# jedisct1/zig-lz4

Measured on AMD Instinct MI355X. Metric: GiB/s uncompressed, block compress+decompress, higher is better.
Workload: dtype u8

## Files before the change

### zig-lz4_amd/csrc/zlz4_compress_dict.hip

```cpp
#include "zlz4_device.hpp"
#include "zlz4_launch.hpp"

namespace zlz4 {

namespace {

__device__ __forceinline__ uint32_t dc_hash4(uint32_t seq) { return (seq * kHashMul) >> 20; }

__device__ __forceinline__ uint32_t dc_skip_sum(uint32_t x) {
    const uint32_t q = x >> 6, r = x & 63u;
    return 32u * q * (q - 1u) + q * r;
}

__device__ __forceinline__ int64_t dc_last_literals(uint8_t *dst, uint32_t dst_len, uint32_t op, const uint8_t *lit_src,
                                                    uint32_t lit, uint32_t lane) {
    if (lit == 0) return (int64_t)op;
    const uint32_t nle = ext_len_bytes(lit);
    if ((uint64_t)op + 1u + nle + lit > dst_len) return kErrOutputTooSmall;
    if (lane == 0) dst[op] = (uint8_t)((lit >= 15u ? 15u : lit) << 4);
    if (lit >= 15u) write_ext_len(dst + op + 1u, lit, lane);
    copy_bytes(dst + op + 1u + nle, lit_src, lit, lane);
    return (int64_t)(op + 1u + nle + lit);
}

// ... 16 lines not shown
    __device__ __forceinline__ uint32_t rd32(uint32_t p) const {
        if (whole(p, 4u)) return ld32(at(p));
        return (uint32_t)byte(p) | (uint32_t)byte(p + 1u) << 8 | (uint32_t)byte(p + 2u) << 16 | (uint32_t)byte(p + 3u) << 24;
    }
};

__device__ __forceinline__ uint32_t dc_extend_match(const VBuf &V, uint32_t m_pos, uint32_t m_cand, uint32_t mlen,
                                                    uint32_t match_limit, uint32_t lane) {
    const uint32_t ip0 = m_pos + kMinMatch, mt0 = m_cand + kMinMatch;
    for (;;) {
        const uint32_t p = ip0 + mlen + lane * 16u;
        uint32_t n = 0;
        if (p < match_limit) n = (match_limit - p) < 16u ? (match_limit - p) : 16u;
        uint32_t d = 0;
        if (n > 0) {
            const uint32_t q = mt0 + mlen + lane * 16u;
            if (p + 16u <= V.end && V.whole(q, 16u)) {
                d = first_diff16(ld128(V.srcv + p), ld128(V.at(q)));
                if (d > n) d = n;
            } else {
                while (d < n && V.srcv[p + d] == V.byte(q + d)) d++;
            }
        }
        const uint64_t stop = ballot(d < 16u);
        if (stop) {
            const uint32_t sl = first_lane(stop);
            return mlen + sl * 16u + rdlane(d, sl);
        }
        mlen += 1024u;
    }
}

}

template <typename T>
__global__ __launch_bounds__(64) void k_compress_fast_dict(
    const uint8_t *d_in, const uint64_t *__restrict__ d_in_off, const uint32_t *__restrict__ d_in_len,
    uint8_t *__restrict__ d_out, const uint64_t *__restrict__ d_out_off, const uint32_t *__restrict__ d_out_cap,
    const uint8_t *d_dict, const uint64_t *__restrict__ d_dict_off, const uint32_t *__restrict__ d_dict_len,
    const uint32_t *__restrict__ d_table, const uint32_t *__restrict__ d_table_idx, int64_t *__restrict__ d_result,
    uint32_t nblocks, uint32_t max_in_len, uint32_t max_dict_len, uint32_t acceleration) {
    extern __shared__ __attribute__((aligned(16))) uint8_t lds_raw[];
    const uint32_t lane = threadIdx.x & 63u;
    const uint32_t blk = blockIdx.x;
    if (blk >= nblocks) return;
    typedef __attribute__((address_space(3))) volatile T lds_entry;
    lds_entry *table = (lds_entry *)lds_raw;

    const uint8_t *src = d_in + d_in_off[blk];
    uint8_t *dst = d_out + d_out_off[blk];
    const uint32_t src_size = rfl(d_in_len[blk]);
    const uint32_t dst_len = rfl(d_out_cap[blk]);
    const uint32_t dict_len = rfl(d_dict_len[blk]);
    const uint32_t D = dict_len < 65536u ? dict_len : 65536u;

    int64_t res;
    if (src_size > kMaxInput) {
        res = kErrInputTooLarge;
    } else if (src_size > max_in_len || D > max_dict_len) {
        res = kErrInvalidState;
    } else if (src_size == 0) {
        res = 0;
    } else if (src_size < kMfLimit + 1u) {
        res = dc_last_literals(dst, dst_len, 0, src, src_size, lane);
    } else {
        VBuf V;
        V.tail = D ? d_dict + d_dict_off[blk] + (dict_len - D) : src;
        V.srcv = src - D;
        V.D = D;
        V.end = D + src_size;
        const uint32_t L = V.end - kMfLimit;
        const uint32_t match_limit = V.end - kLastLiterals;
        {
            const uint32_t tix = d_table_idx ? rfl(d_table_idx[blk]) : blk;
            const u32x4 *seed4 = reinterpret_cast<const u32x4 *>(d_table + (uint64_t)tix * 4096u);
            for (uint32_t k = lane; k < 1024u; k += 64u) {
                const u32x4 v = seed4[k];
                table[4u * k + 0u] = (T)(v.x < L ? v.x : 0u);
                table[4u * k + 1u] = (T)(v.y < L ? v.y : 0u);
                table[4u * k + 2u] = (T)(v.z < L ? v.z : 0u);
                table[4u * k + 3u] = (T)(v.w < L ? v.w : 0u);
            }
            __builtin_amdgcn_fence(__ATOMIC_RELEASE, "wavefront");
        }
        const uint32_t accel = acceleration < 1u ? 1u : (acceleration > 65537u ? 65537u : acceleration);
        const uint32_t cbase = accel > 64u ? accel : 64u;
        const uint32_t s_cbase = dc_skip_sum(cbase);
        const uint64_t lane_bit = 1ull << lane;
        const uint64_t lanes_below = lane_bit - 1ull;

        uint32_t anchor = D, op = 0;
        uint32_t F0 = D > 1u ? D : 1u;
        bool has_ins = false;
        bool failed = false;
        uint32_t guard = 0;
        u32x4 fwd_pf = {0, 0, 0, 0};
        uint32_t pf_anchor = 0xFFFFFFFFu;
        while (F0 < L) {
            if (++guard > src_size) { failed = true; break; }
            int32_t ub = has_ins ? -1 : 0;

            if (accel == 1u && F0 == anchor + 1u && has_ins && (uint64_t)anchor + 192u < L) {
              bool moved = false;
              bool to_generic = false;
              for (;;) {
                const uint32_t A = anchor;
                const uint32_t pos = A + lane;
                const u32x4 fwd = pf_anchor == A ? fwd_pf : ld128(V.srcv + pos);
                const uint32_t prod = fwd.x * kHashMul;
                const uint32_t h = prod >> 20;
                const uint32_t mine = (uint32_t)(T)pos;
                const uint32_t old = table[h];
                const uint64_t okm = ballot(old > 0) & ballot(old < pos) & ballot(old + kMaxDist >= pos);
                const bool old_ok = in_mask(okm);
                u32x4 cold = {0, 0, 0, 0};
                if (old_ok) cold = V.ld128v(old);
                u32x4 f2 = {0, 0, 0, 0}, c2 = f2, f3 = f2, c3 = f2;
                table[h] = (T)mine;
                __builtin_amdgcn_fence(__ATOMIC_RELEASE, "wavefront");
                const uint32_t rb = table[h];
                uint64_t losers = ballot(rb != mine);
                uint64_t grp = lane_bit;
                while (losers) {
                    const uint32_t l = first_lane(losers);
                    const uint32_t hh = rdlane(h, l);
                    const uint64_t same = ballot(h == hh);
                    if (in_mask(same)) grp = same;
                    losers &= ~same;
                }

                const uint64_t vom = okm & ballot(cold.x == fwd.x);
                const bool vo = in_mask(vom);
                uint32_t mlo;
                {
                    const uint32_t x1 = fwd.y ^ cold.y, x2 = fwd.z ^ cold.z, x3 = fwd.w ^ cold.w;
                    const uint32_t xs = x1 ? x1 : (x2 ? x2 : x3);
                    const uint32_t xbase = x1 ? 0u : (x2 ? 4u : 8u);
                    mlo = xs ? xbase + ((uint32_t)__builtin_ctz(xs) >> 3) : 12u;
                }
                const bool need2 = in_mask(vom & ballot(mlo == 12u));
                if (need2) {
                    f2 = ld128(V.srcv + pos + 16u); f3 = ld128(V.srcv + pos + 32u);
                    c2 = V.ld128v(old + 16u); c3 = V.ld128v(old + 32u);
                }
                if (need2) {
                    const uint32_t d2 = first_diff16_sel(f2, c2);
                    mlo += d2 == 16u ? 16u + first_diff16_sel(f3, c3) : d2;
                }
                const uint64_t singm = ballot(lane_rank(grp) == 0u);
                const uint64_t lt44 = ballot(mlo < 44u);
                const uint64_t cfast = vom & lt44;
                const uint64_t nsing = ~singm;
                const uint64_t slow = (nsing & ~cfast) | (vom & ~lt44);
                uint32_t J, S;
                {
                    const uint64_t mj = cfast >> lane, ms = slow >> lane;
                    J = mj ? lane + (uint32_t)__builtin_ctzll(mj) : 64u;
                    S = ms ? lane + (uint32_t)__builtin_ctzll(ms) : 64u;
                }
                uint32_t v_end = lane + kMinMatch + mlo;
                uint32_t mlo_e = mlo, off_e = pos - old;
                uint32_t XP, Q;
                {
                    const uint32_t xm = J < S ? J : S;
                    XP = xm | ((uint32_t)((nsing >> (xm & 63u)) & 1ull) << 7);
                    Q = (vo ? 1u : 0u) | (mlo << 1);
                }
                uint32_t PK;
                {
                    const uint32_t jc = J & 63u;
                    const uint32_t ve_j = shfl(v_end, jc);
                    const bool fastok = J < 64u && S > J && !((nsing >> jc) & 1ull);
                    PK = fastok ? (J | (ve_j << 6)) : 0xFFFFFFFFu;
                }

                uint32_t f = 1;
                uint32_t a = 0;
                uint32_t nseq = 0;
                uint64_t cov_acc = 0;
                bool continue_generic = false;
                const bool tight = dst_len - op < 512u;
                uint32_t a0 = a, op0 = op;
                uint64_t mm_run = 0;
                auto covered_now = [&]() -> uint64_t {
                    if (mm_run == 0) return cov_acc;
                    const uint64_t mb = mm_run & lanes_below;
                    const uint32_t pj = mb ? 63u - (uint32_t)__builtin_clzll(mb) : 0u;
                    const uint32_t pe = shfl(v_end, pj);
                    return cov_acc | ballot(mb != 0 && lane < pe);
                };
                auto flush_run = [&]() {
                    const uint64_t mb = mm_run & lanes_below;
                    const bool has_prev = mb != 0;
                    const uint32_t pj = has_prev ? 63u - (uint32_t)__builtin_clzll(mb) : 0u;
                    const uint32_t pend_all = shfl(v_end, pj);
                    const uint32_t pend = has_prev ? pend_all : a0;
                    const uint64_t covm = ballot(mb != 0) & ballot(lane < pend_all);
                    const bool is_m = in_mask(mm_run);
                    const uint32_t jlast = 63u - (uint32_t)__builtin_clzll(mm_run);
                    const uint64_t litmask = ballot(lane >= a0) & ~(ballot(lane >= jlast) | covm | mm_run);
                    const bool is_lit = in_mask(litmask);
                    const uint64_t extm = mm_run & ballot(mlo_e >= 15u);
                    const uint64_t at_or_above = mm_run & ~lanes_below;
                    const uint32_t my_m = at_or_above ? (uint32_t)__builtin_ctzll(at_or_above) : lane;
                    const uint64_t ownm = ballot(my_m - pend >= 15u);
                    const uint32_t own_l = in_mask(ownm) ? 1u : 0u;
                    const uint64_t lextm = mm_run & ownm;
                    const uint32_t k = lane_rank(mm_run);
                    const uint32_t lb = lane_rank(litmask);
                    const uint32_t o1 = op0 + 3u * k + lb + 1u + lane_rank(extm) + lane_rank(lextm) + own_l;
                    if (is_lit) dst[o1] = (uint8_t)fwd.x;
                    if (is_m) {
                        const uint32_t lit_k = lane - pend;
                        uint8_t *tk = dst + (o1 - 1u - lit_k - own_l);
                        tk[0] = (uint8_t)(((lit_k < 15u ? lit_k : 15u) << 4) | (mlo_e < 15u ? mlo_e : 15u));
                        if (own_l) tk[1] = (uint8_t)(lit_k - 15u);
                        const uint16_t off16 = (uint16_t)off_e;
                        __builtin_memcpy(dst + o1, &off16, 2);
                        if (mlo_e >= 15u) dst[o1 + 2u] = (uint8_t)(mlo_e - 15u);
                    }
                    const uint32_t nm = (uint32_t)__popcll(mm_run);
                    op = op0 + 3u * nm + (uint32_t)__popcll(litmask) + (uint32_t)__popcll(extm) + (uint32_t)__popcll(lextm);
                    cov_acc |= covm;
                    mm_run = 0;
                };
                for (;;) {
                    if (mm_run == 0) { a0 = a; op0 = op; }
                    if (!tight) {
                        uint32_t t_pk, t_j;
#define ZLZ4_FAST_RUN_TRIP                                   \
                            "s_cmp_gt_u32 %[f], 63\n\t"      \
                            "s_cbranch_scc1 3f\n\t"          \
                            "v_readlane_b32 %[pk], %[PK], %[f]\n\t" \
                            "s_cmp_eq_u32 %[pk], -1\n\t"     \
                            "s_cbranch_scc1 3f\n\t"          \
                            "s_lshr_b32 %[a], %[pk], 6\n\t"  \
                            "s_add_u32 %[f], %[a], 1\n\t"    \
                            "s_and_b32 %[j], %[pk], 63\n\t"  \
                            "s_bitset1_b64 %[mm], %[j]\n\t"  \
                            "s_add_u32 %[nseq], %[nseq], 1\n\t"
                        asm volatile(
                            "s_nop 3\n"
                            "1:\n\t"
                            ZLZ4_FAST_RUN_TRIP
                            ZLZ4_FAST_RUN_TRIP
                            "s_branch 1b\n"
                            "3:\n"
                            : [f] "+s"(f), [a] "+s"(a), [nseq] "+s"(nseq), [mm] "+s"(mm_run), [pk] "=&s"(t_pk), [j] "=&s"(t_j)
                            : [PK] "v"(PK)
                            : "scc");
#undef ZLZ4_FAST_RUN_TRIP
                    }
                    if (f >= 64u) {
                        if (nseq == 0u) continue_generic = true;
                        break;
                    }

                    const uint32_t xp = rdlane(XP, f);
                    const uint32_t x = xp & 127u;
                    if (x >= 64u) {
                        if (nseq == 0u) continue_generic = true;
                        break;
                    }
                    uint64_t pm = 0;
                    if (xp >> 7) {
                        const uint64_t grp_x = (uint64_t)rdlane((uint32_t)grp, x) | ((uint64_t)rdlane((uint32_t)(grp >> 32), x) << 32);
                        pm = grp_x & ~covered_now() & ((1ull << x) - 1ull);
                    }
                    const uint32_t j = x;
                    const uint32_t m_pos = A + j;
                    uint32_t m_cand, mlen;
                    if (pm) {
                        const uint32_t pr = 63u - (uint32_t)__builtin_clzll(pm);
                        if (rdlane(fwd.x, pr) != rdlane(fwd.x, x)) { f = x + 1u; continue; }
                        m_cand = A + pr;
                        const uint64_t xa = ((uint64_t)(rdlane(fwd.z, j) ^ rdlane(fwd.z, pr)) << 32) | (rdlane(fwd.y, j) ^ rdlane(fwd.y, pr));
                        const uint32_t xb = rdlane(fwd.w, j) ^ rdlane(fwd.w, pr);
                        if (xa) mlen = (uint32_t)__builtin_ctzll(xa) >> 3;
                        else if (xb) mlen = 8u + ((uint32_t)__builtin_ctz(xb) >> 3);
                        else mlen = dc_extend_match(V, m_pos, m_cand, 12u, match_limit, lane);
                    } else {
                        const uint32_t q = rdlane(Q, x);
                        if (!(q & 1u)) { f = x + 1u; continue; }
                        mlen = q >> 1;
                        if (mlen < 44u && !tight) {
                            mm_run |= 1ull << j;
                            nseq++;
                            a = j + kMinMatch + mlen;
                            if (a >= 64u) break;
                            f = a + 1u;
                            continue;
                        }
                        m_cand = rdlane(old, x);
                        if (mlen >= 44u) mlen = dc_extend_match(V, m_pos, m_cand, 44u, match_limit, lane);
                    }
                    const uint32_t lit = j - a;
                    const uint32_t offset = m_pos - m_cand;
                    const uint32_t e = j + kMinMatch + mlen;
                    if (!tight && mlen < 270u) {
                        v_end = wrlane(e, j, v_end);
                        mlo_e = wrlane(mlen, j, mlo_e);
                        off_e = wrlane(offset, j, off_e);
                        mm_run |= 1ull << j;
                        nseq++;
                        a = e;
                        if (e >= 64u) break;
                        f = e + 1u;
                        continue;
                    }
                    if (mm_run) flush_run();
                    const uint32_t nle = ext_len_bytes(lit), nme = ext_len_bytes(mlen);
                    const uint64_t seq_end = (uint64_t)op + 1u + nle + lit + 2u + nme;
                    if (seq_end > dst_len) { failed = true; break; }
                    if (lane == 0)
                        dst[op] = (uint8_t)(((lit >= 15u ? 15u : lit) << 4) | (mlen >= 15u ? 15u : mlen));
                    if (lit >= 15u) write_ext_len(dst + op + 1u, lit, lane);
                    uint8_t *o = dst + op + 1u + nle;
                    if (lane >= a && lane < j) o[lane - a] = (uint8_t)fwd.x;
                    o += lit;
                    if (lane < 2u) o[lane] = (uint8_t)(offset >> (8u * lane));
                    if (mlen >= 15u) write_ext_len(o + 2u, mlen, lane);
                    op = (uint32_t)seq_end;
                    {
                        const uint64_t upto_e = e >= 64u ? ~0ull : (1ull << e) - 1ull;
                        cov_acc |= upto_e & ~((2ull << j) - 1ull);
                    }
                    nseq++;
                    a = e;
                    if (e >= 64u) break;
                    f = e + 1u;
                }
                const bool next_win = !continue_generic && !failed && a != 0u && (uint64_t)A + a + 192u < L;
                if (next_win) {
                    pf_anchor = A + a;
                    fwd_pf = ld128(V.srcv + pf_anchor + lane);
                }
                if (mm_run && !failed) flush_run();
                anchor = A + a;
                const uint32_t f_end = continue_generic ? 64u : (a >= 64u ? 64u : a + 1u);
                const uint64_t ins = ~cov_acc & (f_end >= 64u ? ~0ull : (1ull << f_end) - 1ull);
                if (failed) break;
                const uint64_t gi = grp & ins;
                const bool put_mine = in_mask(ins) && (gi & ~lanes_below & ~lane_bit) == 0;
                if (put_mine || gi == 0) table[h] = (T)(put_mine ? mine : old);
                __builtin_amdgcn_fence(__ATOMIC_RELEASE, "wavefront");
                moved = anchor != A;
                to_generic = continue_generic;
                if (next_win) {
                    has_ins = true;
                    F0 = anchor + 1u;
                    continue;
                }
                break;
              }
                if (failed) break;
                if (!to_generic && moved) {
                    if (anchor < L) { has_ins = true; F0 = anchor + 1u; }
                    else { has_ins = false; F0 = L; }
                    continue;
                }
                if (to_generic) ub = 63;
            }

            bool found = false;
            uint32_t m_pos = 0, m_cand = 0, m_local = 0;
            bool m_local_done = false;
            for (;;) {
                const int32_t u = ub + (int32_t)lane;
                uint32_t pos, step_next;
                if (u <= 0) {
                    pos = (u < 0) ? F0 - 1u : F0;
                    step_next = accel;
                } else if (u == 1) {
                    pos = F0 + accel;
                    step_next = accel >> 6;
                } else {
                    const uint32_t x = cbase + (uint32_t)u - 1u;
                    pos = F0 + accel + dc_skip_sum(x) - s_cbase;
                    step_next = x >> 6;
                }
                const bool is_probe = u >= 0;
                const bool bail = is_probe && ((uint64_t)pos + step_next > L);
                const uint64_t bail_mask = ballot(bail);
                const uint32_t nb = bail_mask ? first_lane(bail_mask) : 64u;
                const bool active = lane < nb;

                const bool have16 = active && (pos + 16u <= V.end);
                u32x4 fwd = {0, 0, 0, 0};
                if (have16) fwd = ld128(V.srcv + pos);
                else if (active) fwd.x = ld32(V.srcv + pos);
                const uint32_t h = dc_hash4(fwd.x);
                const uint32_t mine = (uint32_t)(T)pos;

                uint32_t old = 0, rb = 0;
                if (active) {
                    old = table[h];
                    table[h] = (T)mine;
                }
                __builtin_amdgcn_fence(__ATOMIC_RELEASE, "wavefront");
                if (active) rb = table[h];
                uint64_t losers = ballot(active && rb != mine);
                uint64_t grp = lane_bit;
                int32_t pred = -1;
                while (losers) {
                    const uint32_t l = first_lane(losers);
                    const uint32_t hh = rdlane(h, l);
                    const uint64_t same = ballot(active && h == hh);
                    if (active && h == hh) {
                        grp = same;
                        const uint64_t below = same & lanes_below;
                        pred = below ? 63 - (int32_t)__clzll((long long)below) : -1;
                    }
                    losers &= ~same;
                }
                const uint32_t pred_pos = shfl(pos, (uint32_t)(pred < 0 ? 0 : pred));
                const uint32_t cand = pred >= 0 ? pred_pos : old;

                bool valid = is_probe && active && cand > 0 && cand < pos && (cand + kMaxDist >= pos);
                u32x4 cnd = {0, 0, 0, 0};
                bool cnd16 = false;
                if (valid) {
                    cnd16 = have16 && V.whole(cand, 16u);
                    if (cnd16) cnd = ld128(V.at(cand)); else cnd.x = V.rd32(cand);
                    valid = cnd.x == fwd.x;
                }
                const uint64_t valid_mask = ballot(valid);

                if (valid_mask) {
                    const uint32_t wl = first_lane(valid_mask);
                    if (active && lane > wl) table[h] = (T)old;
                    __builtin_amdgcn_fence(__ATOMIC_RELEASE, "wavefront");
                    const uint64_t upto = (2ull << wl) - 1ull;
                    if (active && lane <= wl && ((grp & upto & ~lanes_below & ~lane_bit) == 0)) table[h] = (T)mine;
                    __builtin_amdgcn_fence(__ATOMIC_RELEASE, "wavefront");
                    uint32_t loc = 0;
                    bool loc_done = false;
                    if (lane == wl && cnd16) {
                        const uint32_t lim = match_limit - (pos + kMinMatch);
                        u32x4 a = fwd, b = cnd;
                        a.x = 0; b.x = 0;
                        loc = first_diff16(a, b) - 4u;
                        if (loc >= lim) { loc = lim; loc_done = true; }
                        else if (loc < 12u) loc_done = true;
                    }
                    m_pos = rdlane(pos, wl);
                    m_cand = rdlane(cand, wl);
                    m_local = rdlane(loc, wl);
                    m_local_done = rdlane((uint32_t)loc_done, wl) != 0;
                    found = true;
                    break;
                }
                if (bail_mask) break;
                if (active && ((grp & ~lanes_below & ~lane_bit) == 0) && grp != lane_bit) table[h] = (T)mine;
                __builtin_amdgcn_fence(__ATOMIC_RELEASE, "wavefront");
                ub += 64;
            }
            if (!found) break;

            const uint32_t mlen = m_local_done ? m_local : dc_extend_match(V, m_pos, m_cand, m_local, match_limit, lane);

            const uint32_t lit = m_pos - anchor;
            const uint32_t nle = ext_len_bytes(lit), nme = ext_len_bytes(mlen);
            const uint64_t seq_end = (uint64_t)op + 1u + nle + lit + 2u + nme;
            if (seq_end > dst_len) { failed = true; break; }
            if (lane == 0)
                dst[op] = (uint8_t)(((lit >= 15u ? 15u : lit) << 4) | (mlen >= 15u ? 15u : mlen));
            if (lit >= 15u) write_ext_len(dst + op + 1u, lit, lane);
            uint8_t *o = dst + op + 1u + nle;
            copy_bytes(o, V.srcv + anchor, lit, lane);
            o += lit;
            const uint32_t offset = m_pos - m_cand;
            if (lane < 2u) o[lane] = (uint8_t)(offset >> (8u * lane));
            if (mlen >= 15u) write_ext_len(o + 2u, mlen, lane);
            op = (uint32_t)seq_end;

            const uint32_t end = m_pos + kMinMatch + mlen;
            anchor = end;
            if (end < L) { has_ins = true; F0 = end + 1u; }
            else { has_ins = false; F0 = L; }
        }
// ... 27 lines not shown
```

### zig-lz4_amd/csrc/zlz4_compress_fast.hip

```cpp
#include <cstdlib>

#include "zlz4_device.hpp"
#include "zlz4_launch.hpp"

#ifdef ZLZ4_STAMPS
__device__ unsigned long long g_zlz4_stamps[24];
#define STAMP_DECL unsigned long long st_acc[24] = {0,0,0,0,0,0,0,0,0,0,0,0,0,0,0,0,0,0,0,0,0,0,0,0}; unsigned long long st_last = __builtin_amdgcn_s_memtime();
#define STAMP(i) do { unsigned long long st_now; __builtin_amdgcn_sched_barrier(0); \
                      asm volatile("s_memtime %0\n\ts_waitcnt lgkmcnt(0)" : "=s"(st_now) :: "memory"); \
                      __builtin_amdgcn_sched_barrier(0); st_acc[i] += st_now - st_last; st_last = st_now; } while (0)
#define STAMP_COUNT(i) do { st_acc[i] += 1; } while (0)
#define STAMP_FLUSH do { if (lane == 0) for (int st_k = 0; st_k < 24; st_k++) atomicAdd(&g_zlz4_stamps[st_k], st_acc[st_k]); } while (0)
#else
#define STAMP_DECL
#define STAMP(i)
#define STAMP_COUNT(i)
#define STAMP_FLUSH
#endif

namespace zlz4 {

__device__ __forceinline__ uint32_t hash4(uint32_t seq) { return (seq * kHashMul) >> 20; }

__device__ __forceinline__ uint32_t skip_sum(uint32_t x) {
// ... 98 lines not shown
        const uint32_t cbase = accel > 64u ? accel : 64u;
        const uint32_t s_cbase = skip_sum(cbase);
        const uint32_t L = src_size - kMfLimit;
        const uint32_t match_limit = src_size - kLastLiterals;
        const uint64_t lane_bit = 1ull << lane;
        const uint64_t lanes_below = lane_bit - 1ull;

        uint32_t anchor = 0, op = 0;
        uint32_t F0 = 1;
        bool has_ins = false;
        bool failed = false;
        STAMP_DECL
        STAMP(0);

        uint32_t guard = 0;

        constexpr bool kRing = sizeof(T) == 2;
        uint32_t rpos = 0x80000000u + 4u * lane;
        uint32_t r0 = 0, r1 = 0, r2 = 0;
        uint32_t ring_lim = 0;
        if constexpr (kRing) asm volatile("v_mov_b32 %0, %1" : "=v"(ring_lim) : "s"(src_size - 4u));
        auto ring_q = [&](uint32_t q) -> uint32_t { return q < ring_lim ? q : ring_lim; };
        auto ring_sel = [&](uint32_t A, uint32_t &ja) -> uint32_t {
            uint32_t rel = rfl(A - rpos);
            if (rel >= 256u) {
                const bool reload = rel >= 512u;
                const uint32_t nb = reload ? (A & ~127u) + 4u * lane : rpos + 256u;
                asm volatile("s_waitcnt vmcnt(0)\n\t"
                             "s_cmpk_lt_u32 %[rel], 0x200\n\t"
                             "s_cbranch_scc1 1f\n\t"
                             "global_load_dword %[r0], %[q0], %[src]\n\t"
                             "global_load_dword %[r1], %[q1], %[src]\n\t"
                             "s_waitcnt vmcnt(0)\n\t"
                             "s_branch 2f\n"
                             "1:\n\t"
                             "v_mov_b32 %[r0], %[r1]\n\t"
                             "v_mov_b32 %[r1], %[r2]\n"
                             "2:\n\t"
                             "global_load_dword %[r2], %[q2], %[src]"
                             : [r0] "+v"(r0), [r1] "+v"(r1), [r2] "+v"(r2)
                             : [rel] "s"(rel), [q0] "v"(ring_q(nb)), [q1] "v"(ring_q(nb + 256u)), [q2] "v"(ring_q(nb + 512u)),
                               [src] "s"(src)
                             : "scc", "memory");
                rpos = nb;
                rel = reload ? A & 127u : rel - 256u;
            }
            ja = ((rel & ~3u) + (((A & 3u) + lane) & ~3u)) & 0xFFu;
            return lane >= (rel >> 2) ? r0 : r1;
        };
#define ZLZ4_SEL_DWORD(sel, ja, K) ((uint32_t)__builtin_amdgcn_ds_bpermute((int)add_wrap_byte<4u * (K)>(ja), (int)(sel)))
        auto ring_fwd = [&](uint32_t sel, uint32_t ja, uint32_t A, uint32_t &hi4) -> u32x4 {
            const uint32_t sh = (A + lane) & 3u;
            const uint32_t w0 = (uint32_t)__builtin_amdgcn_ds_bpermute((int)ja, (int)sel);
            const uint32_t w1 = ZLZ4_SEL_DWORD(sel, ja, 1), w2 = ZLZ4_SEL_DWORD(sel, ja, 2), w3 = ZLZ4_SEL_DWORD(sel, ja, 3);
            hi4 = ZLZ4_SEL_DWORD(sel, ja, 4);
            return u32x4{__builtin_amdgcn_alignbyte(w1, w0, sh), __builtin_amdgcn_alignbyte(w2, w1, sh),
                         __builtin_amdgcn_alignbyte(w3, w2, sh), __builtin_amdgcn_alignbyte(hi4, w3, sh)};
        };
        auto ring_fwd2 = [&](uint32_t sel, uint32_t ja, uint32_t A, uint32_t hi4, u32x4 &f2, u32x4 &f3) {
            const uint32_t sh = (A + lane) & 3u;
            const uint32_t w5 = ZLZ4_SEL_DWORD(sel, ja, 5), w6 = ZLZ4_SEL_DWORD(sel, ja, 6), w7 = ZLZ4_SEL_DWORD(sel, ja, 7);
            const uint32_t w8 = ZLZ4_SEL_DWORD(sel, ja, 8), w9 = ZLZ4_SEL_DWORD(sel, ja, 9), w10 = ZLZ4_SEL_DWORD(sel, ja, 10);
            const uint32_t w11 = ZLZ4_SEL_DWORD(sel, ja, 11), w12 = ZLZ4_SEL_DWORD(sel, ja, 12);
            f2 = u32x4{__builtin_amdgcn_alignbyte(w5, hi4, sh), __builtin_amdgcn_alignbyte(w6, w5, sh),
                       __builtin_amdgcn_alignbyte(w7, w6, sh), __builtin_amdgcn_alignbyte(w8, w7, sh)};
            f3 = u32x4{__builtin_amdgcn_alignbyte(w9, w8, sh), __builtin_amdgcn_alignbyte(w10, w9, sh),
                       __builtin_amdgcn_alignbyte(w11, w10, sh), __builtin_amdgcn_alignbyte(w12, w11, sh)};
        };
#undef ZLZ4_SEL_DWORD
        u32x4 fwd_pf = {0, 0, 0, 0};
        uint32_t sel_pf = 0, ja_pf = 0, hi4_pf = 0;
        uint32_t pf_anchor = 0xFFFFFFFFu;
        while (F0 < L) {
            if (++guard > src_size) { failed = true; break; }
            int32_t ub = -1;

            if (accel == 1u && F0 == anchor + 1u && has_ins && (uint64_t)anchor + 192u < L) {
              bool moved = false;
              bool to_generic = false;
              for (;;) {
                const uint32_t A = anchor;
                const uint32_t pos = A + lane;
                if (kRing && pf_anchor != A) {
                    sel_pf = ring_sel(A, ja_pf);
                    fwd_pf = ring_fwd(sel_pf, ja_pf, A, hi4_pf);
                }
                const uint32_t sel = sel_pf, ja = ja_pf, hi4 = hi4_pf;
                const u32x4 fwd = (kRing || pf_anchor == A) ? fwd_pf : ld128(src + pos);
                const uint32_t prod = fwd.x * kHashMul;
                const uint32_t h = prod >> 20;
                const uint32_t tg = (prod >> 12) & 0xFFu;
                const uint32_t mine = kTag == 2 ? (pos | (tg << 24)) : (uint32_t)(T)pos;
                STAMP(1);
                STAMP_COUNT(16);
                uint32_t told = tg;
                const uint32_t old_e = table[h];
                if (kTag == 1) told = tags[h];
                if (kTag == 2) told = old_e >> 24;
                const uint32_t old = old_e & kPosMask;
                uint64_t okm = ballot(old > 0) & ballot(old + kMaxDist >= pos);
                if (kSeed) okm &= ballot(old < pos);
                if (kTag != 0) okm &= ballot(told == tg);
                const bool old_ok = in_mask(okm);
                u32x4 cold = {0, 0, 0, 0};
                if (old_ok) cold = ld128(src + old);
                constexpr bool kGuess2 = sizeof(T) == 4;
                const uint32_t old12 = kGuess2 ? shfl(old, (lane + 12u) & 63u) : 0u;
                const bool pred2 = kGuess2 && old_ok && lane < 52u && old12 == old + 12u;
                u32x4 f2 = {0, 0, 0, 0}, c2 = f2, f3 = f2, c3 = f2;
                if (pred2) {
                    if (!kRing) { f2 = ld128(src + pos + 16u); f3 = ld128(src + pos + 32u); }
                    c2 = ld128(src + old + 16u); c3 = ld128(src + old + 32u);
                }
                STAMP(3);
                table[h] = (T)mine;
                __builtin_amdgcn_fence(__ATOMIC_RELEASE, "wavefront");
                const uint32_t rb = table[h];
                uint64_t losers = ballot(rb != mine);
                uint64_t grp = lane_bit;
                while (losers) {
                    const uint32_t l = first_lane(losers);
                    const uint32_t hh = rdlane(h, l);
                    const uint64_t same = ballot(h == hh);
                    if (in_mask(same)) grp = same;
                    losers &= ~same;
                }
                STAMP(2);

                const uint64_t vom = okm & ballot(cold.x == fwd.x);
                const bool vo = in_mask(vom);
                uint32_t mlo;
                {
                    const uint32_t x1 = fwd.y ^ cold.y, x2 = fwd.z ^ cold.z, x3 = fwd.w ^ cold.w;
                    const uint32_t xs = x1 ? x1 : (x2 ? x2 : x3);
                    const uint32_t xbase = x1 ? 0u : (x2 ? 4u : 8u);
                    mlo = xs ? xbase + ((uint32_t)__builtin_ctz(xs) >> 3) : 12u;
                }
                const uint64_t need2m = vom & ballot(mlo == 12u);
                const bool need2 = in_mask(need2m);
                if (need2 && !pred2) {
                    if (!kRing) { f2 = ld128(src + pos + 16u); f3 = ld128(src + pos + 32u); }
                    c2 = ld128(src + old + 16u); c3 = ld128(src + old + 32u);
                }
                if (kRing && need2m) ring_fwd2(sel, ja, A, hi4, f2, f3);
                if (need2) {
                    const uint32_t d2 = first_diff16_sel(f2, c2);
                    mlo += d2 == 16u ? 16u + first_diff16_sel(f3, c3) : d2;
                }
                const uint64_t singm = ballot(lane_rank(grp) == 0u);
                const uint64_t lt44 = ballot(mlo < 44u);
                const uint64_t cfast = vom & lt44;
                const uint64_t nsing = ~singm;
                const uint64_t slow = (nsing & ~cfast) | (vom & ~lt44);
                uint32_t J, S;
                {
                    const uint64_t mj = cfast >> lane, ms = slow >> lane;
                    J = mj ? lane + (uint32_t)__builtin_ctzll(mj) : 64u;
                    S = ms ? lane + (uint32_t)__builtin_ctzll(ms) : 64u;
                }
                uint32_t v_end = lane + kMinMatch + mlo;
                uint32_t mlo_e = mlo, off_e = pos - old;
                uint32_t XP, Q;
                {
                    const uint32_t xm = J < S ? J : S;
                    XP = xm | ((uint32_t)((nsing >> (xm & 63u)) & 1ull) << 7);
                    Q = (vo ? 1u : 0u) | (mlo << 1);
                }
                uint32_t PK;
                {
                    const uint32_t jc = J & 63u;
                    const uint32_t ve_j = shfl(v_end, jc);
                    const bool fastok = J < 64u && S > J && !((nsing >> jc) & 1ull);
                    PK = fastok ? (J | (ve_j << 6)) : 0xFFFFFFFFu;
                }

                STAMP(6);
                uint32_t f = 1;
                uint32_t a = 0;
                uint32_t nseq = 0;
                uint64_t cov_acc = 0;
                bool continue_generic = false;
                const bool tight = dst_len - op < 512u;
                uint32_t a0 = a, op0 = op;
                uint64_t mm_run = 0;
                auto covered_now = [&]() -> uint64_t {
                    if (mm_run == 0) return cov_acc;
                    const uint64_t mb = mm_run & lanes_below;
                    const uint32_t pj = mb ? 63u - (uint32_t)__builtin_clzll(mb) : 0u;
                    const uint32_t pe = shfl(v_end, pj);
                    return cov_acc | ballot(mb != 0 && lane < pe);
                };
                auto flush_run = [&]() {
                    STAMP(9); STAMP_COUNT(21);
                    const uint64_t mb = mm_run & lanes_below;
                    const bool has_prev = mb != 0;
                    const uint32_t pj = has_prev ? 63u - (uint32_t)__builtin_clzll(mb) : 0u;
                    const uint32_t pend_all = shfl(v_end, pj);
                    const uint32_t pend = has_prev ? pend_all : a0;
                    const uint64_t covm = ballot(mb != 0) & ballot(lane < pend_all);
                    const bool is_m = in_mask(mm_run);
                    const uint32_t jlast = 63u - (uint32_t)__builtin_clzll(mm_run);
                    const uint64_t litmask = ballot(lane >= a0) & ~(ballot(lane >= jlast) | covm | mm_run);
                    const bool is_lit = in_mask(litmask);
                    const uint64_t extm = mm_run & ballot(mlo_e >= 15u);
                    const uint64_t at_or_above = mm_run & ~lanes_below;
                    const uint32_t my_m = at_or_above ? (uint32_t)__builtin_ctzll(at_or_above) : lane;
                    const uint64_t ownm = ballot(my_m - pend >= 15u);
                    const uint32_t own_l = in_mask(ownm) ? 1u : 0u;
                    const uint64_t lextm = mm_run & ownm;
                    const uint32_t k = lane_rank(mm_run);
                    const uint32_t lb = lane_rank(litmask);
                    const uint32_t o1 = op0 + 3u * k + lb + 1u + lane_rank(extm) + lane_rank(lextm) + own_l;
                    if (is_lit) dst[o1] = (uint8_t)fwd.x;
                    if (is_m) {
                        const uint32_t lit_k = lane - pend;
                        uint8_t *tk = dst + (o1 - 1u - lit_k - own_l);
                        tk[0] = (uint8_t)(((lit_k < 15u ? lit_k : 15u) << 4) | (mlo_e < 15u ? mlo_e : 15u));
                        if (own_l) tk[1] = (uint8_t)(lit_k - 15u);
                        const uint16_t off16 = (uint16_t)off_e;
                        __builtin_memcpy(dst + o1, &off16, 2);
                        if (mlo_e >= 15u) dst[o1 + 2u] = (uint8_t)(mlo_e - 15u);
                    }
                    const uint32_t nm = (uint32_t)__popcll(mm_run);
                    op = op0 + 3u * nm + (uint32_t)__popcll(litmask) + (uint32_t)__popcll(extm) + (uint32_t)__popcll(lextm);
                    cov_acc |= covm;
                    mm_run = 0;
                    STAMP(10);
                };
                for (;;) {
                    if (mm_run == 0) { a0 = a; op0 = op; }
                    if (!tight) {
                        uint32_t t_pk, t_j;
#define ZLZ4_FAST_RUN_TRIP                                   \
                            "s_cmp_gt_u32 %[f], 63\n\t"      \
                            "s_cbranch_scc1 3f\n\t"          \
                            "v_readlane_b32 %[pk], %[PK], %[f]\n\t" \
                            "s_cmp_eq_u32 %[pk], -1\n\t"     \
                            "s_cbranch_scc1 3f\n\t"          \
                            "s_lshr_b32 %[a], %[pk], 6\n\t"  \
                            "s_add_u32 %[f], %[a], 1\n\t"    \
                            "s_and_b32 %[j], %[pk], 63\n\t"  \
                            "s_bitset1_b64 %[mm], %[j]\n\t"  \
                            "s_add_u32 %[nseq], %[nseq], 1\n\t"
                        asm volatile(
                            "s_nop 3\n"
                            "1:\n\t"
                            ZLZ4_FAST_RUN_TRIP
                            ZLZ4_FAST_RUN_TRIP
                            "s_branch 1b\n"
                            "3:\n"
                            : [f] "+s"(f), [a] "+s"(a), [nseq] "+s"(nseq), [mm] "+s"(mm_run), [pk] "=&s"(t_pk), [j] "=&s"(t_j)
                            : [PK] "v"(PK)
                            : "scc");
#undef ZLZ4_FAST_RUN_TRIP
                    }
                    STAMP(8);
                    if (f >= 64u) {
                        if (nseq == 0u) continue_generic = true;
                        break;
                    }

                    const uint32_t xp = rdlane(XP, f);
                    const uint32_t x = xp & 127u;
                    if (x >= 64u) {
                        if (nseq == 0u) continue_generic = true;
                        break;
                    }
                    uint64_t pm = 0;
                    if (xp >> 7) {
                        const uint64_t grp_x = (uint64_t)rdlane((uint32_t)grp, x) | ((uint64_t)rdlane((uint32_t)(grp >> 32), x) << 32);
                        pm = grp_x & ~covered_now() & ((1ull << x) - 1ull);
                    }
                    const uint32_t j = x;
                    const uint32_t m_pos = A + j;
                    uint32_t m_cand, mlen;
                    if (pm) {
                        const uint32_t pr = 63u - (uint32_t)__builtin_clzll(pm);
                        if (rdlane(fwd.x, pr) != rdlane(fwd.x, x)) { STAMP_COUNT(19); STAMP(9); f = x + 1u; continue; }
                        STAMP_COUNT(18);
                        m_cand = A + pr;
                        const uint64_t xa = ((uint64_t)(rdlane(fwd.z, j) ^ rdlane(fwd.z, pr)) << 32) | (rdlane(fwd.y, j) ^ rdlane(fwd.y, pr));
                        const uint32_t xb = rdlane(fwd.w, j) ^ rdlane(fwd.w, pr);
                        if (xa) mlen = (uint32_t)__builtin_ctzll(xa) >> 3;
                        else if (xb) mlen = 8u + ((uint32_t)__builtin_ctz(xb) >> 3);
                        else mlen = extend_match(src, m_pos, m_cand, 12u, match_limit, src_size, lane);
                    } else {
                        const uint32_t q = rdlane(Q, x);
                        if (!(q & 1u)) { STAMP_COUNT(19); STAMP(9); f = x + 1u; continue; }
                        STAMP_COUNT(18);
                        mlen = q >> 1;
                        if (mlen < 44u && !tight) {
                            mm_run |= 1ull << j;
                            nseq++;
                            a = j + kMinMatch + mlen;
                            STAMP(9);
                            if (a >= 64u) break;
                            f = a + 1u;
                            continue;
                        }
                        m_cand = rdlane(old, x);
                        if (mlen >= 44u) mlen = extend_match(src, m_pos, m_cand, 44u, match_limit, src_size, lane);
                    }
                    const uint32_t lit = j - a;
                    const uint32_t offset = m_pos - m_cand;
                    const uint32_t e = j + kMinMatch + mlen;
                    if (!tight && mlen < 270u) {
                        v_end = wrlane(e, j, v_end);
                        mlo_e = wrlane(mlen, j, mlo_e);
                        off_e = wrlane(offset, j, off_e);
                        mm_run |= 1ull << j;
                        nseq++;
                        a = e;
                        STAMP(9);
                        if (e >= 64u) break;
                        f = e + 1u;
                        continue;
                    }
                    if (mm_run) flush_run();
                    const uint32_t nle = ext_len_bytes(lit), nme = ext_len_bytes(mlen);
                    const uint64_t seq_end = (uint64_t)op + 1u + nle + lit + 2u + nme;
                    if (seq_end > dst_len) { failed = true; break; }
                    if (lane == 0)
                        dst[op] = (uint8_t)(((lit >= 15u ? 15u : lit) << 4) | (mlen >= 15u ? 15u : mlen));
                    if (lit >= 15u) write_ext_len(dst + op + 1u, lit, lane);
                    uint8_t *o = dst + op + 1u + nle;
                    if (lane >= a && lane < j) o[lane - a] = (uint8_t)fwd.x;
                    o += lit;
                    if (lane < 2u) o[lane] = (uint8_t)(offset >> (8u * lane));
                    if (mlen >= 15u) write_ext_len(o + 2u, mlen, lane);
                    op = (uint32_t)seq_end;
                    {
                        const uint64_t upto_e = e >= 64u ? ~0ull : (1ull << e) - 1ull;
                        cov_acc |= upto_e & ~((2ull << j) - 1ull);
                    }
                    nseq++;
                    a = e;
                    if (e >= 64u) break;
                    f = e + 1u;
                }
                const bool next_win = !continue_generic && !failed && a != 0u && (uint64_t)A + a + 192u < L;
                if (next_win) {
                    pf_anchor = A + a;
                    if constexpr (kRing) {
                        sel_pf = ring_sel(pf_anchor, ja_pf);
                        fwd_pf = ring_fwd(sel_pf, ja_pf, pf_anchor, hi4_pf);
                    } else {
                        fwd_pf = ld128(src + pf_anchor + lane);
                    }
                }
                if (mm_run && !failed) flush_run();
                anchor = A + a;
                STAMP(4);
                const uint32_t f_end = continue_generic ? 64u : (a >= 64u ? 64u : a + 1u);
                const uint64_t ins = ~cov_acc & (f_end >= 64u ? ~0ull : (1ull << f_end) - 1ull);
                if (failed) break;
                const uint64_t gi = grp & ins;
                const bool put_mine = in_mask(ins) && (gi & ~lanes_below & ~lane_bit) == 0;
                if (put_mine || gi == 0) table[h] = (T)(put_mine ? mine : old_e);
                if (kTag == 1 && put_mine) tags[h] = (uint8_t)tg;
                __builtin_amdgcn_fence(__ATOMIC_RELEASE, "wavefront");
                STAMP(5);
                moved = anchor != A;
                to_generic = continue_generic;
                if (next_win) {
                    has_ins = true;
                    F0 = anchor + 1u;
                    continue;
                }
                break;
              }
                if (failed) break;
                if (!to_generic && moved) {
                    if (anchor < L) { has_ins = true; F0 = anchor + 1u; }
                    else { has_ins = false; F0 = L; }
                    continue;
                }
                if (to_generic) ub = 63;
            }

            bool found = false, bailed = false;
            uint32_t m_pos = 0, m_cand = 0, m_local = 0;
            bool m_local_done = false;
            for (;;) {
                const int32_t u = ub + (int32_t)lane;
                uint32_t pos, step_next;
                if (u <= 0) {
                    pos = (u < 0) ? F0 - 1u : F0;
                    step_next = accel;
                } else if (u == 1) {
                    pos = F0 + accel;
                    step_next = accel >> 6;
                } else {
                    const uint32_t x = cbase + (uint32_t)u - 1u;
                    pos = F0 + accel + skip_sum(x) - s_cbase;
                    step_next = x >> 6;
                }
                const bool is_probe = u >= 0;
                const bool bail = is_probe && ((uint64_t)pos + step_next > L);
                const uint64_t bail_mask = ballot(bail);
                const uint32_t nb = bail_mask ? first_lane(bail_mask) : 64u;
                const bool active = (lane < nb) && (is_probe || has_ins);

                const bool have16 = active && (pos + 16u <= src_size);
                u32x4 fwd = {0, 0, 0, 0};
                if (have16) fwd = ld128(src + pos);
                else if (active) fwd.x = ld32(src + pos);
                const uint32_t prod = fwd.x * kHashMul;
                const uint32_t h = prod >> 20;
                const uint32_t tg = (prod >> 12) & 0xFFu;
                const uint32_t mine = kTag == 2 ? (pos | (tg << 24)) : (uint32_t)(T)pos;

                uint32_t old_e = 0, rb = 0, told = tg;
                if (active) {
                    old_e = table[h];
                    if (kTag == 1) told = tags[h];
                    table[h] = (T)mine;
                }
                if (kTag == 2) told = old_e >> 24;
                const uint32_t old = old_e & kPosMask;
                __builtin_amdgcn_fence(__ATOMIC_RELEASE, "wavefront");
                if (active) rb = table[h];
                uint64_t losers = ballot(active && rb != mine);
                uint64_t grp = lane_bit;
                int32_t pred = -1;
                while (losers) {
                    const uint32_t l = first_lane(losers);
                    const uint32_t hh = rdlane(h, l);
                    const uint64_t same = ballot(active && h == hh);
                    if (active && h == hh) {
                        grp = same;
                        const uint64_t below = same & lanes_below;
                        pred = below ? 63 - (int32_t)__clzll((long long)below) : -1;
                    }
                    losers &= ~same;
                }
                const uint32_t pred_pos = shfl(pos, (uint32_t)(pred < 0 ? 0 : pred));
                const uint32_t cand = pred >= 0 ? pred_pos : old;

                bool valid = is_probe && active && cand > 0 && cand < pos && (cand + kMaxDist >= pos) &&
                             (kTag == 0 || pred >= 0 || told == tg);
                u32x4 cnd = {0, 0, 0, 0};
                if (valid) {
                    if (have16) cnd = ld128(src + cand); else cnd.x = ld32(src + cand);
                    valid = cnd.x == fwd.x;
                }
                const uint64_t valid_mask = ballot(valid);

                if (valid_mask) {
                    const uint32_t wl = first_lane(valid_mask);
                    if (active && lane > wl) table[h] = (T)old_e;
                    __builtin_amdgcn_fence(__ATOMIC_RELEASE, "wavefront");
                    const uint64_t upto = (2ull << wl) - 1ull;
                    if (active && lane <= wl && ((grp & upto & ~lanes_below & ~lane_bit) == 0)) {
                        table[h] = (T)mine;
                        if (kTag == 1) tags[h] = (uint8_t)tg;
                    }
                    uint32_t loc = 0;
                    bool loc_done = false;
                    if (lane == wl) {
                        const uint32_t lim = match_limit - (pos + kMinMatch);
                        if (have16) {
                            u32x4 a = fwd, b = cnd;
                            a.x = 0; b.x = 0;
                            loc = first_diff16(a, b) - 4u;
                            if (loc >= lim) { loc = lim; loc_done = true; }
                            else if (loc < 12u) loc_done = true;
                        }
                    }
                    m_pos = rdlane(pos, wl);
                    m_cand = rdlane(cand, wl);
                    m_local = rdlane(loc, wl);
                    m_local_done = rdlane((uint32_t)loc_done, wl) != 0;
                    found = true;
                    break;
                }
                if (bail_mask) {
                    if constexpr (kSeed) {
                        if (active && ((grp & ~lanes_below & ~lane_bit) == 0) && grp != lane_bit) table[h] = (T)mine;
                        __builtin_amdgcn_fence(__ATOMIC_RELEASE, "wavefront");
                    }
                    bailed = true; break;
                }
                if (active && ((grp & ~lanes_below & ~lane_bit) == 0)) {
                    if (grp != lane_bit) table[h] = (T)mine;
                    if (kTag == 1) tags[h] = (uint8_t)tg;
                }
                __builtin_amdgcn_fence(__ATOMIC_RELEASE, "wavefront");
                ub += 64;
// ... 156 lines not shown
```

Baseline: 89.96.

## Track match-run ends in a scalar bitmask to replace shuffles and ballots

Adds a scalar 64-bit E_run bitmask that records where each batched match ends. Covered lanes and previous-sequence ends can then come from scalar bit arithmetic, replacing the shfl/ballot cross-lane lookups in flush_run and covered_now. The fast-path inline asm loop is tightened: the packed value gets a sign-bit stop flag so one compare replaces two checks, and the nseq counter is dropped in favour of testing a. This trims scalar and cross-lane work in the hot serial greedy parse, with some risk of subtle edge-case bugs around lane 63 and window boundaries.

After: 92.13 (median of 6 runs). +2.4%, better.

```diff
diff --git a/zig-lz4_amd/csrc/zlz4_compress_dict.hip b/zig-lz4_amd/csrc/zlz4_compress_dict.hip
--- a/zig-lz4_amd/csrc/zlz4_compress_dict.hip
+++ b/zig-lz4_amd/csrc/zlz4_compress_dict.hip
@@ -192,53 +192,41 @@
                 const uint64_t cfast = vom & lt44;
                 const uint64_t nsing = ~singm;
                 const uint64_t slow = (nsing & ~cfast) | (vom & ~lt44);
+                const uint64_t fastm = cfast & singm;
+                const uint64_t stopm = slow | (cfast & nsing);
                 uint32_t J, S;
                 {
-                    const uint64_t mj = cfast >> lane, ms = slow >> lane;
+                    const uint64_t mj = fastm >> lane, ms = stopm >> lane;
                     J = mj ? lane + (uint32_t)__builtin_ctzll(mj) : 64u;
                     S = ms ? lane + (uint32_t)__builtin_ctzll(ms) : 64u;
                 }
-                uint32_t v_end = lane + kMinMatch + mlo;
+                const uint32_t v_end = lane + kMinMatch + mlo;
                 uint32_t mlo_e = mlo, off_e = pos - old;
-                uint32_t XP, Q;
-                {
-                    const uint32_t xm = J < S ? J : S;
-                    XP = xm | ((uint32_t)((nsing >> (xm & 63u)) & 1ull) << 7);
-                    Q = (vo ? 1u : 0u) | (mlo << 1);
-                }
+                const uint32_t X = J < S ? J : S;
+                const uint32_t Q = (mlo << 2) | (in_mask(nsing) ? 2u : 0u) | (vo ? 1u : 0u);
                 uint32_t PK;
                 {
-                    const uint32_t jc = J & 63u;
-                    const uint32_t ve_j = shfl(v_end, jc);
-                    const bool fastok = J < 64u && S > J && !((nsing >> jc) & 1ull);
-                    PK = fastok ? (J | (ve_j << 6)) : 0xFFFFFFFFu;
+                    const uint32_t ve_j = shfl(v_end, J & 63u);
+                    const bool fastok = J < S;
+                    PK = fastok ? (J | ((ve_j + 1u) << 6) | (ve_j >= 63u ? 0x80000000u : 0u)) : 0xFFFFFFFFu;
                 }
 
                 uint32_t f = 1;
                 uint32_t a = 0;
-                uint32_t nseq = 0;
                 uint64_t cov_acc = 0;
                 bool continue_generic = false;
                 const bool tight = dst_len - op < 512u;
-                uint32_t a0 = a, op0 = op;
+                uint32_t a0 = a;
                 uint64_t mm_run = 0;
-                auto covered_now = [&]() -> uint64_t {
-                    if (mm_run == 0) return cov_acc;
-                    const uint64_t mb = mm_run & lanes_below;
-                    const uint32_t pj = mb ? 63u - (uint32_t)__builtin_clzll(mb) : 0u;
-                    const uint32_t pe = shfl(v_end, pj);
-                    return cov_acc | ballot(mb != 0 && lane < pe);
-                };
+                uint64_t E_run = 0;
+                auto covered_now = [&]() -> uint64_t { return cov_acc | (E_run - (mm_run << 1)); };
                 auto flush_run = [&]() {
-                    const uint64_t mb = mm_run & lanes_below;
-                    const bool has_prev = mb != 0;
-                    const uint32_t pj = has_prev ? 63u - (uint32_t)__builtin_clzll(mb) : 0u;
-                    const uint32_t pend_all = shfl(v_end, pj);
-                    const uint32_t pend = has_prev ? pend_all : a0;
-                    const uint64_t covm = ballot(mb != 0) & ballot(lane < pend_all);
+                    const uint64_t covm = E_run - (mm_run << 1);
+                    const uint64_t ends = (E_run | (1ull << a0) | 1ull) & (lanes_below | lane_bit);
+                    const uint32_t pend = 63u - (uint32_t)__builtin_clzll(ends);
                     const bool is_m = in_mask(mm_run);
                     const uint32_t jlast = 63u - (uint32_t)__builtin_clzll(mm_run);
-                    const uint64_t litmask = ballot(lane >= a0) & ~(ballot(lane >= jlast) | covm | mm_run);
+                    const uint64_t litmask = ((1ull << jlast) - 1ull) & ~((1ull << a0) - 1ull) & ~(covm | mm_run);
                     const bool is_lit = in_mask(litmask);
                     const uint64_t extm = mm_run & ballot(mlo_e >= 15u);
                     const uint64_t at_or_above = mm_run & ~lanes_below;
@@ -248,7 +236,7 @@
                     const uint64_t lextm = mm_run & ownm;
                     const uint32_t k = lane_rank(mm_run);
                     const uint32_t lb = lane_rank(litmask);
-                    const uint32_t o1 = op0 + 3u * k + lb + 1u + lane_rank(extm) + lane_rank(lextm) + own_l;
+                    const uint32_t o1 = op + 3u * k + lb + 1u + lane_rank(extm) + lane_rank(lextm) + own_l;
                     if (is_lit) dst[o1] = (uint8_t)fwd.x;
                     if (is_m) {
                         const uint32_t lit_k = lane - pend;
@@ -260,25 +248,24 @@
                         if (mlo_e >= 15u) dst[o1 + 2u] = (uint8_t)(mlo_e - 15u);
                     }
                     const uint32_t nm = (uint32_t)__popcll(mm_run);
-                    op = op0 + 3u * nm + (uint32_t)__popcll(litmask) + (uint32_t)__popcll(extm) + (uint32_t)__popcll(lextm);
+                    op += 3u * nm + (uint32_t)__popcll(litmask) + (uint32_t)__popcll(extm) + (uint32_t)__popcll(lextm);
                     cov_acc |= covm;
                     mm_run = 0;
+                    E_run = 0;
                 };
                 for (;;) {
-                    if (mm_run == 0) { a0 = a; op0 = op; }
-                    if (!tight) {
+                    if (mm_run == 0) a0 = a;
+                    if (!tight && f < 64u) {
                         uint32_t t_pk, t_j;
 #define ZLZ4_FAST_RUN_TRIP                                   \
-                            "s_cmp_gt_u32 %[f], 63\n\t"      \
+                            "v_readlane_b32 %[pk], %[PK], %[f]\n\t" \
+                            "s_cmp_lt_i32 %[pk], 0\n\t"      \
                             "s_cbranch_scc1 3f\n\t"          \
-                            "v_readlane_b32 %[pk], %[PK], %[f]\n\t" \
-                            "s_cmp_eq_u32 %[pk], -1\n\t"     \
-                            "s_cbranch_scc1 3f\n\t"          \
-                            "s_lshr_b32 %[a], %[pk], 6\n\t"  \
-                            "s_add_u32 %[f], %[a], 1\n\t"    \
+                            "s_lshr_b32 %[f], %[pk], 6\n\t"  \
                             "s_and_b32 %[j], %[pk], 63\n\t"  \
                             "s_bitset1_b64 %[mm], %[j]\n\t"  \
-                            "s_add_u32 %[nseq], %[nseq], 1\n\t"
+                            "s_sub_u32 %[a], %[f], 1\n\t"    \
+                            "s_bitset1_b64 %[er], %[a]\n\t"
                         asm volatile(
                             "s_nop 3\n"
                             "1:\n\t"
@@ -286,24 +273,30 @@
                             ZLZ4_FAST_RUN_TRIP
                             "s_branch 1b\n"
                             "3:\n"
-                            : [f] "+s"(f), [a] "+s"(a), [nseq] "+s"(nseq), [mm] "+s"(mm_run), [pk] "=&s"(t_pk), [j] "=&s"(t_j)
+                            : [f] "+s"(f), [a] "+s"(a), [mm] "+s"(mm_run), [er] "+s"(E_run), [pk] "=&s"(t_pk), [j] "=&s"(t_j)
                             : [PK] "v"(PK)
                             : "scc");
 #undef ZLZ4_FAST_RUN_TRIP
+                        if (t_pk != 0xFFFFFFFFu) {
+                            mm_run |= 1ull << (t_pk & 63u);
+                            f = (t_pk >> 6) & 127u;
+                            a = f - 1u;
+                            if (a == 63u) E_run |= 1ull << 63;
+                        }
                     }
                     if (f >= 64u) {
-                        if (nseq == 0u) continue_generic = true;
+                        if (a == 0u) continue_generic = true;
                         break;
                     }
 
-                    const uint32_t xp = rdlane(XP, f);
-                    const uint32_t x = xp & 127u;
+                    const uint32_t x = rdlane(X, f);
                     if (x >= 64u) {
-                        if (nseq == 0u) continue_generic = true;
+                        if (a == 0u) continue_generic = true;
                         break;
                     }
+                    const uint32_t q = rdlane(Q, x);
                     uint64_t pm = 0;
-                    if (xp >> 7) {
+                    if (q & 2u) {
                         const uint64_t grp_x = (uint64_t)rdlane((uint32_t)grp, x) | ((uint64_t)rdlane((uint32_t)(grp >> 32), x) << 32);
                         pm = grp_x & ~covered_now() & ((1ull << x) - 1ull);
                     }
@@ -320,13 +313,12 @@
                         else if (xb) mlen = 8u + ((uint32_t)__builtin_ctz(xb) >> 3);
                         else mlen = dc_extend_match(V, m_pos, m_cand, 12u, match_limit, lane);
                     } else {
-                        const uint32_t q = rdlane(Q, x);
                         if (!(q & 1u)) { f = x + 1u; continue; }
-                        mlen = q >> 1;
+                        mlen = q >> 2;
                         if (mlen < 44u && !tight) {
                             mm_run |= 1ull << j;
-                            nseq++;
                             a = j + kMinMatch + mlen;
+                            if (a < 64u) E_run |= 1ull << a;
                             if (a >= 64u) break;
                             f = a + 1u;
                             continue;
@@ -338,11 +330,10 @@
                     const uint32_t offset = m_pos - m_cand;
                     const uint32_t e = j + kMinMatch + mlen;
                     if (!tight && mlen < 270u) {
-                        v_end = wrlane(e, j, v_end);
                         mlo_e = wrlane(mlen, j, mlo_e);
                         off_e = wrlane(offset, j, off_e);
                         mm_run |= 1ull << j;
-                        nseq++;
+                        if (e < 64u) E_run |= 1ull << e;
                         a = e;
                         if (e >= 64u) break;
                         f = e + 1u;
@@ -365,7 +356,6 @@
                         const uint64_t upto_e = e >= 64u ? ~0ull : (1ull << e) - 1ull;
                         cov_acc |= upto_e & ~((2ull << j) - 1ull);
                     }
-                    nseq++;
                     a = e;
                     if (e >= 64u) break;
                     f = e + 1u;
diff --git a/zig-lz4_amd/csrc/zlz4_compress_fast.hip b/zig-lz4_amd/csrc/zlz4_compress_fast.hip
--- a/zig-lz4_amd/csrc/zlz4_compress_fast.hip
+++ b/zig-lz4_amd/csrc/zlz4_compress_fast.hip
@@ -274,55 +274,43 @@
                 const uint64_t cfast = vom & lt44;
                 const uint64_t nsing = ~singm;
                 const uint64_t slow = (nsing & ~cfast) | (vom & ~lt44);
+                const uint64_t fastm = cfast & singm;
+                const uint64_t stopm = slow | (cfast & nsing);
                 uint32_t J, S;
                 {
-                    const uint64_t mj = cfast >> lane, ms = slow >> lane;
+                    const uint64_t mj = fastm >> lane, ms = stopm >> lane;
                     J = mj ? lane + (uint32_t)__builtin_ctzll(mj) : 64u;
                     S = ms ? lane + (uint32_t)__builtin_ctzll(ms) : 64u;
                 }
-                uint32_t v_end = lane + kMinMatch + mlo;
+                const uint32_t v_end = lane + kMinMatch + mlo;
                 uint32_t mlo_e = mlo, off_e = pos - old;
-                uint32_t XP, Q;
-                {
-                    const uint32_t xm = J < S ? J : S;
-                    XP = xm | ((uint32_t)((nsing >> (xm & 63u)) & 1ull) << 7);
-                    Q = (vo ? 1u : 0u) | (mlo << 1);
-                }
+                const uint32_t X = J < S ? J : S;
+                const uint32_t Q = (mlo << 2) | (in_mask(nsing) ? 2u : 0u) | (vo ? 1u : 0u);
                 uint32_t PK;
                 {
-                    const uint32_t jc = J & 63u;
-                    const uint32_t ve_j = shfl(v_end, jc);
-                    const bool fastok = J < 64u && S > J && !((nsing >> jc) & 1ull);
-                    PK = fastok ? (J | (ve_j << 6)) : 0xFFFFFFFFu;
+                    const uint32_t ve_j = shfl(v_end, J & 63u);
+                    const bool fastok = J < S;
+                    PK = fastok ? (J | ((ve_j + 1u) << 6) | (ve_j >= 63u ? 0x80000000u : 0u)) : 0xFFFFFFFFu;
                 }
 
                 STAMP(6);
                 uint32_t f = 1;
                 uint32_t a = 0;
-                uint32_t nseq = 0;
                 uint64_t cov_acc = 0;
                 bool continue_generic = false;
                 const bool tight = dst_len - op < 512u;
-                uint32_t a0 = a, op0 = op;
+                uint32_t a0 = a;
                 uint64_t mm_run = 0;
-                auto covered_now = [&]() -> uint64_t {
-                    if (mm_run == 0) return cov_acc;
-                    const uint64_t mb = mm_run & lanes_below;
-                    const uint32_t pj = mb ? 63u - (uint32_t)__builtin_clzll(mb) : 0u;
-                    const uint32_t pe = shfl(v_end, pj);
-                    return cov_acc | ballot(mb != 0 && lane < pe);
-                };
+                uint64_t E_run = 0;
+                auto covered_now = [&]() -> uint64_t { return cov_acc | (E_run - (mm_run << 1)); };
                 auto flush_run = [&]() {
                     STAMP(9); STAMP_COUNT(21);
-                    const uint64_t mb = mm_run & lanes_below;
-                    const bool has_prev = mb != 0;
-                    const uint32_t pj = has_prev ? 63u - (uint32_t)__builtin_clzll(mb) : 0u;
-                    const uint32_t pend_all = shfl(v_end, pj);
-                    const uint32_t pend = has_prev ? pend_all : a0;
-                    const uint64_t covm = ballot(mb != 0) & ballot(lane < pend_all);
+                    const uint64_t covm = E_run - (mm_run << 1);
+                    const uint64_t ends = (E_run | (1ull << a0) | 1ull) & (lanes_below | lane_bit);
+                    const uint32_t pend = 63u - (uint32_t)__builtin_clzll(ends);
                     const bool is_m = in_mask(mm_run);
                     const uint32_t jlast = 63u - (uint32_t)__builtin_clzll(mm_run);
-                    const uint64_t litmask = ballot(lane >= a0) & ~(ballot(lane >= jlast) | covm | mm_run);
+                    const uint64_t litmask = ((1ull << jlast) - 1ull) & ~((1ull << a0) - 1ull) & ~(covm | mm_run);
                     const bool is_lit = in_mask(litmask);
                     const uint64_t extm = mm_run & ballot(mlo_e >= 15u);
                     const uint64_t at_or_above = mm_run & ~lanes_below;
@@ -332,7 +320,7 @@
                     const uint64_t lextm = mm_run & ownm;
                     const uint32_t k = lane_rank(mm_run);
                     const uint32_t lb = lane_rank(litmask);
-                    const uint32_t o1 = op0 + 3u * k + lb + 1u + lane_rank(extm) + lane_rank(lextm) + own_l;
+                    const uint32_t o1 = op + 3u * k + lb + 1u + lane_rank(extm) + lane_rank(lextm) + own_l;
                     if (is_lit) dst[o1] = (uint8_t)fwd.x;
                     if (is_m) {
                         const uint32_t lit_k = lane - pend;
@@ -344,26 +332,25 @@
                         if (mlo_e >= 15u) dst[o1 + 2u] = (uint8_t)(mlo_e - 15u);
                     }
                     const uint32_t nm = (uint32_t)__popcll(mm_run);
-                    op = op0 + 3u * nm + (uint32_t)__popcll(litmask) + (uint32_t)__popcll(extm) + (uint32_t)__popcll(lextm);
+                    op += 3u * nm + (uint32_t)__popcll(litmask) + (uint32_t)__popcll(extm) + (uint32_t)__popcll(lextm);
                     cov_acc |= covm;
                     mm_run = 0;
+                    E_run = 0;
                     STAMP(10);
                 };
                 for (;;) {
-                    if (mm_run == 0) { a0 = a; op0 = op; }
-                    if (!tight) {
+                    if (mm_run == 0) a0 = a;
+                    if (!tight && f < 64u) {
                         uint32_t t_pk, t_j;
 #define ZLZ4_FAST_RUN_TRIP                                   \
-                            "s_cmp_gt_u32 %[f], 63\n\t"      \
+                            "v_readlane_b32 %[pk], %[PK], %[f]\n\t" \
+                            "s_cmp_lt_i32 %[pk], 0\n\t"      \
                             "s_cbranch_scc1 3f\n\t"          \
-                            "v_readlane_b32 %[pk], %[PK], %[f]\n\t" \
-                            "s_cmp_eq_u32 %[pk], -1\n\t"     \
-                            "s_cbranch_scc1 3f\n\t"          \
-                            "s_lshr_b32 %[a], %[pk], 6\n\t"  \
-                            "s_add_u32 %[f], %[a], 1\n\t"    \
+                            "s_lshr_b32 %[f], %[pk], 6\n\t"  \
                             "s_and_b32 %[j], %[pk], 63\n\t"  \
                             "s_bitset1_b64 %[mm], %[j]\n\t"  \
-                            "s_add_u32 %[nseq], %[nseq], 1\n\t"
+                            "s_sub_u32 %[a], %[f], 1\n\t"    \
+                            "s_bitset1_b64 %[er], %[a]\n\t"
                         asm volatile(
                             "s_nop 3\n"
                             "1:\n\t"
@@ -371,25 +358,31 @@
                             ZLZ4_FAST_RUN_TRIP
                             "s_branch 1b\n"
                             "3:\n"
-                            : [f] "+s"(f), [a] "+s"(a), [nseq] "+s"(nseq), [mm] "+s"(mm_run), [pk] "=&s"(t_pk), [j] "=&s"(t_j)
+                            : [f] "+s"(f), [a] "+s"(a), [mm] "+s"(mm_run), [er] "+s"(E_run), [pk] "=&s"(t_pk), [j] "=&s"(t_j)
                             : [PK] "v"(PK)
                             : "scc");
 #undef ZLZ4_FAST_RUN_TRIP
+                        if (t_pk != 0xFFFFFFFFu) {
+                            mm_run |= 1ull << (t_pk & 63u);
+                            f = (t_pk >> 6) & 127u;
+                            a = f - 1u;
+                            if (a == 63u) E_run |= 1ull << 63;
+                        }
                     }
                     STAMP(8);
                     if (f >= 64u) {
-                        if (nseq == 0u) continue_generic = true;
+                        if (a == 0u) continue_generic = true;
                         break;
                     }
 
-                    const uint32_t xp = rdlane(XP, f);
-                    const uint32_t x = xp & 127u;
+                    const uint32_t x = rdlane(X, f);
                     if (x >= 64u) {
-                        if (nseq == 0u) continue_generic = true;
+                        if (a == 0u) continue_generic = true;
                         break;
                     }
+                    const uint32_t q = rdlane(Q, x);
                     uint64_t pm = 0;
-                    if (xp >> 7) {
+                    if (q & 2u) {
                         const uint64_t grp_x = (uint64_t)rdlane((uint32_t)grp, x) | ((uint64_t)rdlane((uint32_t)(grp >> 32), x) << 32);
                         pm = grp_x & ~covered_now() & ((1ull << x) - 1ull);
                     }
@@ -407,14 +400,13 @@
                         else if (xb) mlen = 8u + ((uint32_t)__builtin_ctz(xb) >> 3);
                         else mlen = extend_match(src, m_pos, m_cand, 12u, match_limit, src_size, lane);
                     } else {
-                        const uint32_t q = rdlane(Q, x);
                         if (!(q & 1u)) { STAMP_COUNT(19); STAMP(9); f = x + 1u; continue; }
                         STAMP_COUNT(18);
-                        mlen = q >> 1;
+                        mlen = q >> 2;
                         if (mlen < 44u && !tight) {
                             mm_run |= 1ull << j;
-                            nseq++;
                             a = j + kMinMatch + mlen;
+                            if (a < 64u) E_run |= 1ull << a;
                             STAMP(9);
                             if (a >= 64u) break;
                             f = a + 1u;
@@ -427,11 +419,10 @@
                     const uint32_t offset = m_pos - m_cand;
                     const uint32_t e = j + kMinMatch + mlen;
                     if (!tight && mlen < 270u) {
-                        v_end = wrlane(e, j, v_end);
                         mlo_e = wrlane(mlen, j, mlo_e);
                         off_e = wrlane(offset, j, off_e);
                         mm_run |= 1ull << j;
-                        nseq++;
+                        if (e < 64u) E_run |= 1ull << e;
                         a = e;
                         STAMP(9);
                         if (e >= 64u) break;
@@ -455,7 +446,6 @@
                         const uint64_t upto_e = e >= 64u ? ~0ull : (1ull << e) - 1ull;
                         cov_acc |= upto_e & ~((2ull << j) - 1ull);
                     }
-                    nseq++;
                     a = e;
                     if (e >= 64u) break;
                     f = e + 1u;
```
